# zkemail/zkemail.rs

Measured on AMD Instinct MI355X. Metric: emails verified/sec (witness gen), higher is better.
Workload: dtype u32; 1 GPU; BASELINE configs[1]: batch 1024 e-mails, 4 KB body, RSA-2048, DKIM-only verify_email; body_bytes=4096, rsa_bits=2048, algo=rsa-sha256, inputs=HBM-resident raw e-mails, batches_in_flight=22, collective=none

## Files before the change

### bindings/zkemail-amd-sys/src/lib.rs

```rust
#![allow(non_camel_case_types, non_upper_case_globals)]

use core::ffi::{c_char, c_int, c_void};

pub const ZKE_OK: u32 = 0;
pub const ZKE_PARSE_FAIL: u32 = 1;
pub const ZKE_KEY_DECODE_FAIL: u32 = 2;
pub const ZKE_DKIM_ERROR: u32 = 3;
pub const ZKE_DKIM_NOT_PASS: u32 = 4;
pub const ZKE_EXTERNAL_INPUT_NULL: u32 = 5;
pub const ZKE_CANON_FAIL: u32 = 6;
pub const ZKE_DFA_DECODE_FAIL: u32 = 7;
pub const ZKE_HEADER_REGEX_FAIL: u32 = 8;
pub const ZKE_BODY_REGEX_FAIL: u32 = 9;
pub const ZKE_UNSUPPORTED: u32 = 10;
pub const ZKE_BODY_DECODE_FAIL: u32 = 11;
pub const ZKE_D_NONE: u32 = 0;
pub const ZKE_D_NEUTRAL: u32 = 1;
pub const ZKE_D_SIG_SYNTAX: u32 = 2;
pub const ZKE_D_MISSING_TAG: u32 = 3;
pub const ZKE_D_INCOMPATIBLE_VERSION: u32 = 4;
pub const ZKE_D_DOMAIN_MISMATCH: u32 = 5;
pub const ZKE_D_FROM_NOT_SIGNED: u32 = 6;
pub const ZKE_D_BAD_QUERY_METHOD: u32 = 7;
pub const ZKE_D_BAD_CANON: u32 = 8;
// ... 437 lines not shown
    pub fn zke_select_keys(e: *mut zke_engine, emails: *const zke_email_ref, n: u32, cand_off: *const u32, keys: *const zke_key_ref, out: *mut zke_result, chosen: *mut u32) -> c_int;
    pub fn zke_select_keys_async(e: *mut zke_engine, emails: *const zke_email_ref, n: u32, cand_off: *const u32, keys: *const zke_key_ref, out: *mut zke_result, chosen: *mut u32, ticket: *mut u64) -> c_int;
    pub fn zke_decode_key_records(e: *mut zke_engine, recs: *const zke_keyrec_ref, m: u32, mode: u32, out: *mut zke_keyrec_out) -> c_int;
    pub fn zke_decode_key_records_async(e: *mut zke_engine, recs: *const zke_keyrec_ref, m: u32, mode: u32, out: *mut zke_keyrec_out, ticket: *mut u64) -> c_int;
    pub fn zke_select_keys_from_records(e: *mut zke_engine, emails: *const zke_email_ref, n: u32, cand_off: *const u32, recs: *const zke_keyrec_ref, mode: u32, out: *mut zke_result, chosen: *mut u32, keys_out: *mut zke_keyrec_out) -> c_int;
    pub fn zke_select_keys_from_records_async(e: *mut zke_engine, emails: *const zke_email_ref, n: u32, cand_off: *const u32, recs: *const zke_keyrec_ref, mode: u32, out: *mut zke_result, chosen: *mut u32, keys_out: *mut zke_keyrec_out, ticket: *mut u64) -> c_int;
    pub fn zke_extract_bodies(e: *mut zke_engine, emails: *const zke_email_ref, n: u32, flags: u32, out: *mut zke_body_out) -> c_int;
    pub fn zke_extract_bodies_async(e: *mut zke_engine, emails: *const zke_email_ref, n: u32, flags: u32, out: *mut zke_body_out, ticket: *mut u64) -> c_int;
    pub fn zke_verify_batch_device(e: *mut zke_engine, r#in: *const zke_batch, raw_total: u64, domain_total: u64, key_total: u64, out_dev: *mut zke_result, stream: *mut c_void) -> c_int;
    pub fn zke_engine_sync(e: *mut zke_engine) -> c_int;
    pub fn zke_engine_join(e: *mut zke_engine, stream: *mut c_void) -> c_int;
    pub fn zke_get_timings(e: *mut zke_engine, t: *mut zke_timings) -> c_int;
    pub fn zke_get_slot_timings(e: *mut zke_engine, slot: u32, t: *mut zke_timings) -> c_int;
    pub fn zke_engine_sha_ring(e: *mut zke_engine) -> c_int;
    pub fn zke_engine_sha_twin(e: *mut zke_engine) -> c_int;
    pub fn zke_set_timing(e: *mut zke_engine, enabled: c_int) -> c_int;
    pub fn zke_verify_email(e: *mut zke_engine, raw: *const u8, raw_len: usize, from_domain: *const c_char, domain_len: usize, key: *const u8, key_len: usize, key_type: u32, external_input_null: u32, out: *mut zke_result) -> c_int;
    pub fn zke_verify_email_with_regex(e: *mut zke_engine, raw: *const u8, raw_len: usize, from_domain: *const c_char, domain_len: usize, key: *const u8, key_len: usize, key_type: u32, external_input_null: u32, header_parts: *const zke_regex_part, n_header_parts: u32, body_parts: *const zke_regex_part, n_body_parts: u32, out: *mut zke_result) -> c_int;
    pub fn zke_wire_decode(format: u32, bytes: *const u8, len: usize, with_regex: u32, out: *mut *mut zke_wire_doc, consumed: *mut usize) -> c_int;
    pub fn zke_wire_free(d: *mut zke_wire_doc);
    pub fn zke_wire_view(d: *const zke_wire_doc, out: *mut zke_wire_email) -> c_int;
    pub fn zke_wire_external_input(d: *const zke_wire_doc, i: u32, name: *mut *const u8, name_len: *mut usize, value: *mut *const u8, value_len: *mut usize, is_null: *mut u32) -> c_int;
    pub fn zke_verify_wire(e: *mut zke_engine, format: u32, bytes: *const u8, len: usize, with_regex: u32, out: *mut zke_result) -> c_int;
    pub fn zke_shard_bounds(raw_off: *const u64, n: u32, world: u32, bounds: *mut u32) -> c_int;
    pub fn zke_sha256_batch(e: *mut zke_engine, msg_blob: *const u8, off: *const u64, n: u32, digests: *mut u8) -> c_int;
    pub fn zke_rsa_modexp_batch(e: *mut zke_engine, sig: *const u8, r#mod: *const u8, exp: *const u64, bytes: u32, n: u32, em: *mut u8, ok: *mut u8) -> c_int;
    pub fn zke_ed25519_verify_batch(e: *mut zke_engine, keys: *const u8, msgs: *const u8, msg_len: u32, sigs: *const u8, n: u32, out: *mut u32) -> c_int;
    pub fn zke_sha256_batch_device(e: *mut zke_engine, msg_blob_dev: *const u8, off_dev: *const u64, n: u32, digests_dev: *mut u8, stream: *mut c_void) -> c_int;
    pub fn zke_abi_encode(from_domain_hash: *const u8, public_key_hash: *const u8, external_inputs: *const *const u8, external_input_lens: *const usize, n_external_inputs: u32, with_matches: u32, matches: *const *const u8, match_lens: *const usize, n_matches: u32, out: *mut u8, out_cap: usize, out_len: *mut usize) -> c_int;
    pub fn zke_version() -> *const c_char;
// ... 5 lines not shown
```

### include/zkemail_amd.h

```cpp
#ifndef ZKEMAIL_AMD_H
#define ZKEMAIL_AMD_H

#include <stddef.h>
#include <stdint.h>

#ifdef __cplusplus
extern "C" {
#endif

enum {
  ZKE_OK                  = 0,
  ZKE_PARSE_FAIL          = 1,
  ZKE_KEY_DECODE_FAIL     = 2,
  ZKE_DKIM_ERROR          = 3,
  ZKE_DKIM_NOT_PASS       = 4,
  ZKE_EXTERNAL_INPUT_NULL = 5,
  ZKE_CANON_FAIL          = 6,
  ZKE_DFA_DECODE_FAIL     = 7,
  ZKE_HEADER_REGEX_FAIL   = 8,
  ZKE_BODY_REGEX_FAIL     = 9,
  ZKE_UNSUPPORTED         = 10,
  ZKE_BODY_DECODE_FAIL    = 11
};

// ... 353 lines not shown
  uint8_t*       bytes; size_t bytes_cap;
  size_t infos_need, bytes_need;
} zke_body_out;
int zke_extract_bodies(zke_engine* e, const zke_email_ref* emails, uint32_t n, uint32_t flags, zke_body_out* out);
int zke_extract_bodies_async(zke_engine* e, const zke_email_ref* emails, uint32_t n, uint32_t flags, zke_body_out* out, uint64_t* ticket);

int zke_verify_batch_device(zke_engine* e, const zke_batch* in, uint64_t raw_total,
                            uint64_t domain_total, uint64_t key_total,
                            zke_result* out_dev, void* stream);
int zke_engine_sync(zke_engine* e);
int zke_engine_join(zke_engine* e, void* stream);
int zke_get_timings(zke_engine* e, zke_timings* t);
int zke_get_slot_timings(zke_engine* e, uint32_t slot, zke_timings* t);
int zke_engine_sha_ring(zke_engine* e);
int zke_engine_sha_twin(zke_engine* e);
int zke_set_timing(zke_engine* e, int enabled);

int zke_verify_email(zke_engine* e, const uint8_t* raw, size_t raw_len,
                     const char* from_domain, size_t domain_len,
                     const uint8_t* key, size_t key_len, uint32_t key_type,
                     uint32_t external_input_null, zke_result* out);

typedef struct zke_regex_part {
  const uint8_t* fwd; size_t fwd_len;
  const uint8_t* bwd; size_t bwd_len;
  uint32_t n_captures;
  const uint8_t* const* captures;
  const size_t* capture_lens;
} zke_regex_part;

// ... 57 lines not shown
```

### zkemail.rs_amd/csrc/canon.hip.h

```cpp
#pragma once
#include "parse.hip.h"
#include <type_traits>

namespace zke {

__device__ __forceinline__ uint32_t ld_coherent_u8(const uint8_t* p) {
  return (uint32_t)__hip_atomic_load(p, __ATOMIC_RELAXED, __HIP_MEMORY_SCOPE_AGENT);
}

template <class LD>
__device__ __forceinline__ uint32_t trailing_crlf_pairs(LD load, uint32_t len, bool* ended = nullptr) {
  uint32_t matched = 0, pos = len;
  if (ended) *ended = false;
  while (pos > 0) {
    const uint32_t lo = pos > 64 ? pos - 64 : 0;
    const uint32_t l = lo + lane_id();
    bool bad = false;
    if (l < pos) {
      const uint32_t c = load(l);
      bad = c != (((len - 1 - l) & 1) ? (uint32_t)'\r' : (uint32_t)'\n');
    }
    const uint64_t m = __ballot(bad);
    if (m) { matched += (pos - 1) - (lo + 63u - (uint32_t)__builtin_clzll(m)); if (ended) *ended = true; break; }
    matched += pos - lo;
    pos = lo;
  }
  return matched / 2;
}

constexpr uint32_t CANON_LDS_TRASH = 3504, CANON_LDS_BYTES = 3504 + 64;
static_assert(CANON_LDS_BYTES <= PARSE_STAGE_BYTES, "the front end lends its staging buffer to the canonicaliser");
__device__ __forceinline__ void canon_body_wave(const BatchDev& B, uint32_t i, uint32_t mode, uint32_t flags, uint32_t boff,
                                                uint32_t blen, uint64_t len_tag, uint8_t* lds, bool ignore_l, bool bucket,
                                                uint32_t hdr_len) {
  const int lane = lane_id();
  EmailMeta* M = B.meta + i;
  zke_result* R = B.results + i;
  const uint64_t r0 = B.raw_off[i];
  const uint32_t raw_len = (uint32_t)(B.raw_off[i + 1] - r0);
  const uint8_t* body = B.raw + r0 + boff;
  uint8_t* regB = B.scratch + scratch_offset(r0 - B.raw_off[0], i) + (((size_t)raw_len + PRE_SLACK + 15) & ~(size_t)15);
  uint32_t full = 0, src_is_raw = 0;

  if (!(flags & ZKE_F_BODY_RELAXED)) {
    if (blen == 0) {
      if (lane < 2) regB[lane] = lane ? '\n' : '\r';
      full = 2;
    } else {
      const uint32_t m = trailing_crlf_pairs([&](uint32_t l) { return (uint32_t)body[l]; }, blen);
      full = m >= 2 ? blen - 2 * (m - 1) : blen;
      src_is_raw = 1;
    }
  } else {
    typedef uint32_t __attribute__((aligned(1))) u32_unaligned;
    typedef uint4 __attribute__((aligned(1))) uint4_store_unaligned;
    auto load4 = [&](uint32_t pos) -> uint32_t {
// ... 166 lines not shown
        }
        __builtin_amdgcn_fence(__ATOMIC_RELEASE, "wavefront");
        __builtin_amdgcn_wave_barrier();
        o += fill;
        fill = 0;
      }
    }
    if (!tail_done) {
      __builtin_amdgcn_fence(__ATOMIC_RELEASE, "agent");
      const uint32_t m = trailing_crlf_pairs([&](uint32_t l) { return ld_coherent_u8(regB + l); }, o);
      if (m >= 2) o -= 2 * (m - 1);
      else if (o > 0 && m == 0) { if (lane < 2) regB[o + lane] = lane ? '\n' : '\r'; o += 2; }
    }
    full = o;
  }
  uint32_t hashed = full;
  if ((flags & ZKE_F_HAS_LENGTH) && !ignore_l) {
    if (len_tag < hashed) hashed = (uint32_t)len_tag;
  }
  if (lane == 0) {
    M->canon_full_len = full; M->hashed_len = hashed; M->body_src_is_raw = src_is_raw;
    if (mode == 0) {
      R->canon_body_len = hashed;
      ShaJob j; j.src = (uint64_t)(src_is_raw ? body : regB); j.dst = (uint64_t)R->body_hash; j.len = hashed;
      j.pad = (flags & ZKE_F_SHA1) ? 1u : 0u;
      B.sha[i] = j;
    }
  }
  if (bucket && lane < 2) sha_bucket(B.order, (uint32_t)lane, B.n_pad, i, lane ? hdr_len : hashed);
}

struct FinArgs { BatchDev b; uint32_t round, max_rounds; uint32_t* pending; uint32_t debug_skip_rsa; };

constexpr uint32_t META_WORDS = sizeof(EmailMeta) / 4;
static_assert(sizeof(EmailMeta) % 16 == 0 && offsetof(EmailMeta, bh) % 4 == 0, "EmailMeta is read as 16-byte words (hipMalloc aligns the array)");
static_assert(offsetof(zke_result, header_hash) == offsetof(zke_result, body_hash) + 32, "the two hashes are read as one run of 16 words");
struct VerdictIn {
  uint32_t m[META_WORDS];
  uint32_t hash[16];
  uint32_t ext_null;
};
#define ZKE_MW(field) (offsetof(EmailMeta, field) / 4)
__device__ __forceinline__ void verdict_load(const EmailMeta* M, const zke_result* R, const uint8_t* ext, VerdictIn& V) {
  const uint4* mp = reinterpret_cast<const uint4*>(M);
// ... 90 lines not shown
```

### zkemail.rs_amd/csrc/engine.hip

```cpp
#include <hip/hip_runtime.h>
#include <hip/hip_ext.h>

#include <algorithm>
#include <atomic>
#include <cstddef>
#include <cstdio>
#include <cstdlib>
#include <cstring>
#include <ctime>
#include <mutex>
#include <shared_mutex>
#include <string>
#include <unordered_map>
#include <vector>

#include "zkemail_amd.h"
#include "sha256.hip.h"
#include "rsa.hip.h"
#include "parse.hip.h"
#include "regex.hip.h"
#include "capture.hip.h"
#include "qpmap.hip.h"
#include "sigscan.hip.h"
#include "keyrec.hip.h"
// ... 375 lines not shown
  delete e;
}

int zke_engine_sha_ring(zke_engine* e) {
  if (!e) return ZKE_E_ARG;
  std::shared_lock<std::shared_mutex> sh(e->big);
  return sha_takes_ring(e->stage) ? 1 : 0;
}

int zke_engine_sha_twin(zke_engine* e) {
  if (!e) return ZKE_E_ARG;
  std::shared_lock<std::shared_mutex> sh(e->big);
  return sha_takes_twin(e->stage) ? 1 : 0;
}

const char* zke_last_error(const zke_engine* e) { (void)e; return g_err.c_str(); }

int zke_engine_join(zke_engine* e, void* stream) {
  if (!e) return ZKE_E_ARG;
  std::shared_lock<std::shared_mutex> sh(e->big);
  HIPCHK(e, hipSetDevice(e->device));
  hipStream_t s = (hipStream_t)stream;
  for (Slot* w : e->slots) {
    std::lock_guard<std::mutex> g(w->mu);
    if (!w->last_stream) continue;
    if (w->last_stream == w->stream) {
      if (s == w->stream) continue;
      HIPCHK(e, hipEventRecord(w->done, w->stream));
    } else if (w->last_stream == s) {
      continue;
// ... 164 lines not shown
```

### zkemail.rs_amd/csrc/parse.hip.h

```cpp
#pragma once
#include <hip/hip_runtime.h>
#include <stdint.h>

#include "zkemail_amd.h"
#include "rsa.hip.h"
#include "sha256.hip.h"
#include "bytes.hip.h"
#include "taglist.hip.h"
#include "hdrsplit.hip.h"
#include "keydec.hip.h"

namespace zke {

struct EmailMeta {
  uint32_t state;
  uint32_t status, detail;
  uint32_t unsupported;
  uint32_t last_touched_sig;
  uint32_t cand_total;
  uint32_t cand_sig_index;
  uint32_t cand_hdr;
  uint32_t cand_err;
  uint32_t post_err;
  uint32_t pre_err;
// ... 89 lines not shown
  uint32_t debug_stop;
  uint32_t strict;
  uint64_t now;
  const KeyCacheEntry* cache;
  uint32_t route_mask;
  uint32_t* wave_count;
  uint32_t* wave_list;
};

#ifdef ZKE_DEV_KNOBS
#define ZKE_DEV_STOP(k) do { if (A.debug_stop == (k)) return; } while (0)
#else
#define ZKE_DEV_STOP(k) do { } while (0)
#endif

__device__ __forceinline__ void canon_body_wave(const BatchDev& B, uint32_t i, uint32_t mode, uint32_t flags, uint32_t boff,
                                                uint32_t blen, uint64_t len_tag, uint8_t* lds, bool ignore_l, bool bucket,
                                                uint32_t hdr_len = 0);
__device__ __forceinline__ void sha_bucket(uint32_t* order, uint32_t kind, uint32_t n_pad, uint32_t i, uint32_t len) {
  const uint32_t cls = sha_len_class((len + 9 + 63) >> 6);
  order[sha_order_key(kind, n_pad) + i] = (cls << 24) | (atomicAdd(order + sha_order_cnt(kind) + cls, 1u) & 0xFFFFFFu);
}


template <bool FAST = true, int MODE = 0>
__device__ __forceinline__ void parse_email(const ParseArgs& A, const uint32_t i, ParseLds& L) {
  const BatchDev& B = A.b;
  const int lane = lane_id();
  EmailMeta* M = B.meta + i;
  zke_result* R = B.results + i;
  RsaJob* J = B.rsa + i;
  const uint32_t round = A.round;
  if (round > 0 && MODE == 0) {
    if (lane < 4) { ShaJob z{0, 0, 0, 0}; B.sha[(size_t)lane * B.n_pad + i] = z; }
    if (lane == 0) J->flags = 0;
    if (M->state != ST_PENDING) return;
  }

  const uint64_t r0 = B.raw_off[i], r1 = B.raw_off[i + 1];
  if (round == 0 && MODE == 0) batch_prologue(B, i, lane == 0, i == 0, (uint32_t)lane, 64);
  Str raw = mkstr(B.raw + r0, (uint32_t)(r1 - r0));
// ... 157 lines not shown
      auto next_occurrence = [&](uint32_t from, uint32_t skip_at) -> uint32_t {
        for (uint32_t base = from; base + bl <= v.len; base += 64) {
          const uint32_t p = base + lane;
          bool cand = p + bl <= v.len && p != skip_at;
          for (uint32_t t = 0; t < fl && cand; t++) cand = ldb(v, p + t) == ldb(v, b_rs + t);
          uint64_t m = __ballot(cand);
          while (m) {
            const uint32_t q = base + (uint32_t)__builtin_ctzll(m);
            m &= m - 1;
            if (same_bytes(v, q, b_rs, bl)) return q;
          }
        }
        return NONE;
      };
      if (!(A.strict & ZKE_STRICT_B_OWN_SPAN) && next_occurrence(0, b_rs) != NONE) {
        uint32_t pos = 0;
        while (pos < v.len) {
          const uint32_t q = next_occurrence(pos, NONE);
          const uint32_t end = (q == NONE) ? v.len : q;
          for (uint32_t base = pos; base < end; base += 64) { const uint32_t l = base + (uint32_t)lane; if (l < end) tmp[tn + (l - pos)] = (uint8_t)ldb(v, l); }
          tn += end - pos;
          if (q == NONE) break;
          pos = q + bl;
        }
        __builtin_amdgcn_fence(__ATOMIC_RELEASE, "agent");
        __builtin_amdgcn_fence(__ATOMIC_ACQUIRE, "agent");
        copied = true;
      }
    }
    Str sv = v;
    if (copied) sv = mkstr(tmp, tn);
    else if (bl) { sv.len = v.len - bl; sv.cut = b_rs; sv.skip = bl; }
    ZKE_DEV_STOP(6);
    Out out{regA, 0, capA, false};
    const bool hrel = (flags & ZKE_F_HDR_RELAXED) != 0;
    const uint32_t hks_lane = hn.ks, hnl_lane = hn.nl;
    {
      const uint8_t* h = L.tagbuf + tagf(L, TG_H, 2);
      const uint32_t hl = tagf(L, TG_H, 3);
      const bool one_win = hl <= 64;
      const uint64_t colons = one_win ? __ballot((uint32_t)lane < hl && h[(uint32_t)lane < hl ? lane : 0] == ':') : 0ull;
      auto colon_after = [&](uint32_t from) -> uint32_t {
        if (one_win) { const uint64_t m = colons & bits_from(from); return m ? (uint32_t)__builtin_ctzll(m) : hl; }
        for (uint32_t base = from & ~63u; base < hl; base += 64) {
          const uint32_t l = base + (uint32_t)lane;
          const uint64_t m = __ballot(l < hl && l >= from && h[l] == ':');
          if (m) return base + (uint32_t)__builtin_ctzll(m);
        }
// ... 70 lines not shown
  if (!have_cand) {
    if (lane == 0) R->sig_index = last_touched;
    if (unsupported) finish(ZKE_UNSUPPORTED, unsupported);
    else finish(ZKE_DKIM_NOT_PASS, err_all ? err_all : (round == 0 ? ZKE_D_NEUTRAL : M->cand_err));
    return;
  }
  ZKE_DEV_STOP(7);
  if (lane == 0) {
    M->state = ST_CAND;
    const uint32_t jf = (cand_flags & ZKE_F_ED25519) ? 0u : (RSA_F_ACTIVE | ((cand_flags & ZKE_F_SHA1) ? (uint32_t)RSA_F_SHA1 : 0u) |
                                                                  (A.route_mask ? M->rsa_route & RSA_F_GROUPS : 0u));
    J->flags = jf;
    M->em_ok = 0;
    if ((jf & RSA_F_ACTIVE) && !(jf & RSA_F_GROUPS) && A.wave_list) A.wave_list[atomicAdd(A.wave_count, 1u)] = i;
  }
  canon_body_wave(B, i, 0, cand_flags, body_off, raw.len - body_off, cand_len_tag, L.stage, false, bucket, cand_hdr_len);
}

#ifndef ZKE_PARSE_PRIO
#define ZKE_PARSE_PRIO 3
#endif
#ifndef ZKE_PARSE_WAVES
#define ZKE_PARSE_WAVES 5
#endif
#ifndef ZKE_PARSE_WG_WAVES
#define ZKE_PARSE_WG_WAVES 1
#endif
constexpr size_t PARSE_DYN_LDS = ZKE_PARSE_WG_WAVES > 1 ? ZKE_PARSE_WG_WAVES * sizeof(ParseLds) : 0;
#ifdef ZKE_PARSE_NUM_VGPR
#define ZKE_PARSE_VGPR_ATTR __attribute__((amdgpu_num_vgpr(ZKE_PARSE_NUM_VGPR)))
#else
#define ZKE_PARSE_VGPR_ATTR
#endif
__global__ __launch_bounds__(64 * ZKE_PARSE_WG_WAVES, ZKE_PARSE_WAVES) ZKE_PARSE_VGPR_ATTR void parse_kernel(ParseArgs A) {
#if ZKE_PARSE_WG_WAVES > 1
  extern __shared__ __attribute__((aligned(16))) uint8_t parse_lds_raw[];
  ParseLds* L = reinterpret_cast<ParseLds*>(parse_lds_raw);
#else
  __shared__ ParseLds L[1];
#endif
  const uint32_t wave = ZKE_PARSE_WG_WAVES > 1 ? __builtin_amdgcn_readfirstlane(threadIdx.x >> 6) : 0;
  const uint32_t email = blockIdx.x * ZKE_PARSE_WG_WAVES + wave;
  if (email >= A.b.n) return;
  if (ZKE_PARSE_PRIO) __builtin_amdgcn_s_setprio(ZKE_PARSE_PRIO);
  parse_email(A, email, L[wave]);
}

__global__ void sha_jobs_from_csr_kernel(const uint8_t* blob, const uint64_t* off, uint32_t n, uint8_t* digests, ShaJob* jobs) {
  uint32_t i = blockIdx.x * blockDim.x + threadIdx.x;
  if (i >= n) return;
  ShaJob j;
  j.src = (uint64_t)(blob + off[i]);
  j.dst = (uint64_t)(digests + (size_t)i * 32);
  j.len = (uint32_t)(off[i + 1] - off[i]);
  j.pad = 0;
  jobs[i] = j;
}

}
```

### zkemail.rs_amd/csrc/pipeline.hip.h

```cpp
#pragma once

namespace {

struct StageTimer {
  Slot* w; hipStream_t s; bool on;
  StageTimer(zke_engine* e_, Slot* w_, hipStream_t s_) : w(w_), s(s_), on(e_->timing.load()) {}
  void mark(int k) { if (on && hipEventRecord(w->ev[k], s) == hipSuccess) w->marks |= 1u << k; }
};

int ensure_zeroed(DevBuf& b, size_t need, hipStream_t s) {
  const void* old = b.p;
  if (int r = b.ensure(need)) return r;
  if (b.p != old && hipMemsetAsync(b.p, 0, b.cap, s) != hipSuccess) return ZKE_E_DEVICE;
  return 0;
}

int ensure_workspace(zke_engine* e, Slot& w, uint32_t n, uint64_t raw_total, bool with_regex, uint32_t P, bool want_em, hipStream_t s) {
  const uint32_t n_pad = (n + 63) & ~63u;
  int r = 0;
  const size_t scratch_bytes = 2 * (size_t)raw_total + (size_t)(n + 1) * SCR_PER_EMAIL + 256;
  if ((r = w.meta.ensure((size_t)n * sizeof(EmailMeta))) || (r = w.rsa_jobs.ensure((size_t)n * sizeof(RsaJob))) ||
      (r = w.sha_jobs.ensure((size_t)4 * n_pad * sizeof(ShaJob))) || (r = w.rsa_ok.ensure((size_t)n * 4)) ||
      (r = ensure_zeroed(w.sha_order, (size_t)2 * (SHA_ORDER_KIND_WORDS + n_pad) * 4, s)) ||
      (r = w.scratch_off.ensure((size_t)(n + 1) * 16)) || (r = w.scratch.ensure(scratch_bytes)))
// ... 178 lines not shown
  B.n_pad = n_pad;
  B.scratch = w.scratch.as<uint8_t>();
  B.scratch_off = scratch_off;
  B.clean_off = clean_off;
  B.pending = w.pending.as<uint32_t>();
  B.meta_verify = nullptr;
  B.order = n < (1u << 24) ? w.sha_order.as<uint32_t>() : nullptr;

  const uint32_t rounds = e->opt.max_sig_rounds;
  const StagePlan plan = plan_stage(e->stage, n, 4 * n_pad, key_total > (uint64_t)n * 272, B.order != nullptr, __atomic_load_n(w.wave_feedback, __ATOMIC_RELAXED));
  {
    const uint32_t round = 0;
    uint32_t* wave_count = w.pending.as<uint32_t>() + 2;
    uint32_t* wave_list = w.rsa_ok.as<uint32_t>();
    ParseArgs pa{B, round, 0, e->debug_parse_stop, e->strict, now, e->key_cache.as<KeyCacheEntry>(), plan.route_mask, wave_count, wave_list};
    hipLaunchKernelGGL(parse_kernel, dim3((n + ZKE_PARSE_WG_WAVES - 1) / ZKE_PARSE_WG_WAVES), dim3(64 * ZKE_PARSE_WG_WAVES), PARSE_DYN_LDS, s, pa);
    tm.mark(MK_FRONT);
    if (!(e->debug_skip_launch & 1) &&
        (r = launch_hash_modexp(e, plan, B.sha, 4 * n_pad, B.rsa, n, B.meta, want_em ? w.em_dbg.as<uint8_t>() : nullptr, wave_count, wave_list, B.order, s)))
      return r;
    tm.mark(MK_HASH);
    EdVerdictArgs va{FinArgs{B, round, rounds, w.pending.as<uint32_t>(), e->debug_skip_rsa}, e->debug_skip_ed, wave_count,
                     e->key_cache.as<KeyCacheEntry>(), want_em ? w.em_dbg.as<uint8_t>() : nullptr, e->strict, now, w.wave_feedback};
    if (!(e->debug_skip_launch & 2)) hipLaunchKernelGGL(ed_verdict_kernel, dim3((n + VERDICT_EMAILS_PER_WAVE - 1) / VERDICT_EMAILS_PER_WAVE), dim3(64), 0, s, va);
    tm.mark(MK_VERDICT);
  }
  HIPCHK(e, hipGetLastError());

  if (in->with_regex) {
    PartInfo parts_small[16];
    std::vector<PartInfo> parts_big;
// ... 258 lines not shown
```

### zkemail.rs_amd/csrc/stage_plan.hip.h

```cpp
#pragma once
#include <stdint.h>
#include <stdlib.h>

#ifdef __HIP__
#define ZKE_PLAN_FN __host__ __device__ inline
#else
#define ZKE_PLAN_FN inline
#endif

namespace zke {

constexpr uint32_t ROUTE_QUAD = 1u;
constexpr uint32_t ROUTE_OCT = 2u;
constexpr uint32_t ROUTE_OCT9 = 4u;

enum class ShaRoutine : uint32_t {
  TWIN,
  RING,
  PAIR,
  BATCH,
};
constexpr uint32_t SHA_TWIN_WIDTH = 32;
ZKE_PLAN_FN uint32_t sha_routine_width(ShaRoutine r) {
  return r == ShaRoutine::BATCH ? 256u : r == ShaRoutine::TWIN ? SHA_TWIN_WIDTH : 64u;
// ... 12 lines not shown
  uint32_t kind = 0;
  for (; kind + 1 < SHA_KINDS; kind++) {
    const uint32_t g = sha_kind_groups(n_pad, twin_kinds, kind);
    if (b < g) break;
    b -= g;
  }
  return kind;
}

struct StageEnv {
  uint32_t slots = 0;
  uint32_t hw_queues = 4;
  int rsa_oct9 = -1;
  int sha_ring = -1;
  int sha_twin = -1;
  uint32_t twin_kinds = 3;
  uint32_t rsa_quad_min = 256;
  uint32_t rsa_oct_min = 128;
  uint32_t sha_mapping = 0;
  uint32_t rsa_lane_groups = 0;
  bool key_cache = false;
};

inline void stage_env_from_environment(StageEnv& v) {
  auto forced = [](const char* name, int& f) { if (const char* s = getenv(name)) f = atoi(s) != 0 ? 1 : 0; };
  const char* q = getenv("GPU_MAX_HW_QUEUES");
  const int hwq = q ? atoi(q) : 0;
  v.hw_queues = hwq > 0 ? (uint32_t)hwq : 4u;
  forced("ZKE_RSA_OCT9", v.rsa_oct9);
  forced("ZKE_SHA_RING", v.sha_ring);
  forced("ZKE_SHA_TWIN", v.sha_twin);
  if (const char* tk = getenv("ZKE_SHA_TWIN_KINDS")) v.twin_kinds = (uint32_t)atoi(tk) & 3u;
#ifdef ZKE_DEV_KNOBS
  if (const char* rm = getenv("ZKE_RSA_QUAD_MIN")) v.rsa_quad_min = (uint32_t)atoi(rm);
  if (const char* ro = getenv("ZKE_RSA_OCT_MIN")) v.rsa_oct_min = (uint32_t)atoi(ro);
#endif
}

inline uint32_t plan_min(uint32_t a, uint32_t b) { return a < b ? a : b; }
inline uint32_t plan_max(uint32_t a, uint32_t b) { return a > b ? a : b; }

constexpr uint32_t CHAIN_BOUND_IN_FLIGHT = 4;
inline bool chain_bound(const StageEnv& v) { return plan_min(v.slots, v.hw_queues) <= CHAIN_BOUND_IN_FLIGHT; }

constexpr uint32_t SHA_PAIR_MAX_GROUPS = 512;
inline bool sha_takes_pairs(const StageEnv& v, uint32_t groups) { return v.sha_mapping ? v.sha_mapping == 2 : groups <= SHA_PAIR_MAX_GROUPS; }
inline bool sha_takes_ring(const StageEnv& v) { return v.sha_ring >= 0 ? v.sha_ring == 1 : chain_bound(v); }
inline bool sha_takes_twin(const StageEnv& v) { return sha_takes_ring(v) && v.sha_twin != 0; }

inline uint32_t rsa_route_mask(const StageEnv& v, uint32_t n, bool any_big) {
  if (!v.key_cache || v.rsa_lane_groups == 1) return 0;
  const bool always = v.rsa_lane_groups == 2;
  const bool oct9 = v.rsa_oct9 >= 0 ? v.rsa_oct9 == 1 : !always && chain_bound(v);
  uint32_t m = 0;
  if (always || n >= v.rsa_quad_min) m |= oct9 ? ROUTE_OCT9 : ROUTE_QUAD;
  if (any_big && (always || n >= v.rsa_oct_min)) m |= ROUTE_OCT;
  return m;
}

struct ShaPlan { ShaRoutine routine; uint32_t grid; };
inline ShaPlan plan_sha(const StageEnv& v, uint32_t n) {
  const ShaRoutine r = !sha_takes_pairs(v, (n + 63) / 64) ? ShaRoutine::BATCH
                       : sha_takes_twin(v)               ? ShaRoutine::TWIN
                       : sha_takes_ring(v)               ? ShaRoutine::RING
                                                         : ShaRoutine::PAIR;
  const uint32_t w = sha_routine_width(r);
  return ShaPlan{r, (n + w - 1) / w};
}

#ifndef ZKE_WAVE_ROLE_MAX_GROUPS
#define ZKE_WAVE_ROLE_MAX_GROUPS 128
#endif
#ifndef ZKE_WAVE_ROLE_MIN_GROUPS
#define ZKE_WAVE_ROLE_MIN_GROUPS 8
#endif

struct StagePlan {
  uint32_t route_mask;
  ShaPlan front;
  ShaRoutine routine;
  uint32_t twin_kinds;
  uint32_t g_sha, g_wave, g_quad, g_oct, g_oct9;
  uint32_t grid() const { return g_sha + g_wave + g_quad + g_oct + g_oct9; }
};
inline StagePlan plan_stage(const StageEnv& v, uint32_t n, uint32_t n_sha, bool any_big, bool have_order, uint32_t last_wave_jobs) {
  StagePlan p{};
  p.route_mask = rsa_route_mask(v, n, any_big);
  const uint32_t want = last_wave_jobs == 0xFFFFFFFFu ? ZKE_WAVE_ROLE_MAX_GROUPS
                                                      : plan_max(ZKE_WAVE_ROLE_MIN_GROUPS, (plan_min(last_wave_jobs, n) + 1) / 2);
  p.g_wave = plan_min((n + 1) / 2, plan_min(want, ZKE_WAVE_ROLE_MAX_GROUPS));
  p.g_quad = (p.route_mask & ROUTE_QUAD) ? (n + 31) / 32 : 0;
  p.g_oct = (p.route_mask & ROUTE_OCT) ? (n + 15) / 16 : 0;
  p.g_oct9 = (p.route_mask & ROUTE_OCT9) ? (n + 15) / 16 : 0;
  p.routine = ShaRoutine::PAIR;
  const uint32_t groups = (n_sha + 63) / 64;
  if (!sha_takes_pairs(v, groups)) { p.front = plan_sha(v, n_sha); return p; }
  if (have_order && sha_takes_twin(v)) p.twin_kinds = v.twin_kinds;
  p.g_sha = p.twin_kinds ? sha_stage_groups(n_sha / 4, p.twin_kinds) : groups;
  if (p.g_sha) p.routine = p.twin_kinds ? ShaRoutine::TWIN : sha_takes_ring(v) ? ShaRoutine::RING : ShaRoutine::PAIR;
  return p;
}

// ... 2 lines not shown
```

### zkemail.rs_amd/engine.py

```python
from __future__ import annotations

import ctypes as C
import os
from typing import Callable, Dict, List, NamedTuple, Optional, Sequence, Tuple

import numpy as np

from . import _abi as A
from ._abi import (CompiledRegex, DebugBuffers, Email, EmailVerifierOutput, EmailWithRegex,
                   EmailWithRegexVerifierOutput, PackedBatch)

_PKG = os.path.dirname(os.path.abspath(__file__))
_LIB_PATH = os.environ.get("ZKE_LIB") or os.path.join(_PKG, "libzkemail_amd.so")
_lib = None


class EngineError(RuntimeError):
    """The C-ABI call itself failed (bad arguments, no device, library missing)."""


class VerifyPanic(AssertionError):

    def __init__(self, status: int, detail: int, index: int = 0):
        self.status, self.detail, self.index = status, detail, index
# ... 129 lines not shown
    lib.zke_select_keys_from_records.argtypes = [vp, erp, C.c_uint32, vp, krp, C.c_uint32, vp, vp, kop]
    lib.zke_select_keys_from_records.restype = C.c_int
    lib.zke_select_keys_from_records_async.argtypes = [vp, erp, C.c_uint32, vp, krp, C.c_uint32, vp, vp, kop, C.POINTER(C.c_uint64)]
    lib.zke_select_keys_from_records_async.restype = C.c_int
    bop = C.POINTER(A.zke_body_out)
    lib.zke_extract_bodies.argtypes = [vp, erp, C.c_uint32, C.c_uint32, bop]
    lib.zke_extract_bodies.restype = C.c_int
    lib.zke_extract_bodies_async.argtypes = [vp, erp, C.c_uint32, C.c_uint32, bop, C.POINTER(C.c_uint64)]
    lib.zke_extract_bodies_async.restype = C.c_int
    if hasattr(lib, "zke_engine_sha_ring"):
        lib.zke_engine_sha_ring.argtypes = [vp]
        lib.zke_engine_sha_ring.restype = C.c_int
    if hasattr(lib, "zke_engine_sha_twin"):
        lib.zke_engine_sha_twin.argtypes = [vp]
        lib.zke_engine_sha_twin.restype = C.c_int
    lib.zke_version.argtypes = []
    lib.zke_version.restype = C.c_char_p
    lib.zke_device_available.argtypes = []
    lib.zke_device_available.restype = C.c_int
    if path is None:
        _lib = lib
    return lib


EXPORTED_SYMBOLS = [
    "zke_engine_create", "zke_engine_destroy", "zke_last_error", "zke_dfa_register", "zke_verify_batch",
    "zke_verify_batch_device", "zke_engine_sync", "zke_get_timings", "zke_set_timing", "zke_verify_email",
    "zke_sha256_batch", "zke_sha256_batch_device", "zke_rsa_modexp_batch", "zke_version", "zke_device_available",
    "zke_ed25519_verify_batch", "zke_engine_reserve", "zke_get_slot_timings", "zke_verify_email_with_regex",
    "zke_abi_encode", "zke_engine_join", "zke_verify_batch_async", "zke_batch_wait", "zke_dfa_status", "zke_dfa_unregister",
    "zke_process_init", "zke_abi_version", "zke_engine_reserve_host", "zke_wire_decode", "zke_wire_free", "zke_wire_view",
    "zke_wire_external_input", "zke_verify_wire", "zke_shard_bounds", "zke_status_name", "zke_verify_emails", "zke_verify_emails_async",
    "zke_verify_emails_with_regex", "zke_verify_emails_with_regex_async",
    "zke_capture_validate", "zke_capture_register", "zke_capture_status", "zke_capture_unregister", "zke_extract_captures",
    "zke_extract_captures_async", "zke_capture_batch",
    "zke_scan_signatures", "zke_scan_signatures_async", "zke_select_keys", "zke_select_keys_async",
    "zke_decode_key_records", "zke_decode_key_records_async", "zke_select_keys_from_records", "zke_select_keys_from_records_async",
    "zke_engine_sha_ring", "zke_engine_sha_twin",
    "zke_qp_clean_batch", "zke_extract_captures_mapped", "zke_extract_captures_mapped_async",
    "zke_extract_bodies", "zke_extract_bodies_async",
]


class SigInfo(NamedTuple):
    header_index: int
    code: int
    algo: int
    selector: bytes
    value_span: Tuple[int, int]


class SigScan(NamedTuple):
    status: int
# ... 409 lines not shown
        self._check(self.lib.zke_engine_reserve_host(self.h, max_n, max_input_bytes), "zke_engine_reserve_host")

    def sync(self):
        self._check(self.lib.zke_engine_sync(self.h), "zke_engine_sync")

    def sha_ring(self) -> bool:
        r = self.lib.zke_engine_sha_ring(self.h)
        self._check(min(r, 0), "zke_engine_sha_ring")
        return r == 1

    def sha_twin(self) -> bool:
        r = self.lib.zke_engine_sha_twin(self.h)
        self._check(min(r, 0), "zke_engine_sha_twin")
        return r == 1

    def join(self, stream: int = 0):
        self._check(self.lib.zke_engine_join(self.h, stream), "zke_engine_join")

    def slot_timings(self, slot: int) -> dict:
        t = A.zke_timings()
        self._check(self.lib.zke_get_slot_timings(self.h, slot, C.byref(t)), "zke_get_slot_timings")
        return {k: getattr(t, k) for k, _ in A.zke_timings._fields_}

    def set_timing(self, on: bool):
        self._check(self.lib.zke_set_timing(self.h, 1 if on else 0), "zke_set_timing")

    def timings(self) -> dict:
        t = A.zke_timings()
        self._check(self.lib.zke_get_timings(self.h, C.byref(t)), "zke_get_timings")
        return {k: getattr(t, k) for k, _ in A.zke_timings._fields_}
# ... 274 lines not shown
```

Before: 16.27 million emails/s.

## Add a helper wave that canonicalises the body while the main wave parses headers

Measured after the change: 17.34 million emails/s, median of 6. +6.6%, better.

```diff
diff --git a/bindings/zkemail-amd-sys/src/lib.rs b/bindings/zkemail-amd-sys/src/lib.rs
--- a/bindings/zkemail-amd-sys/src/lib.rs
+++ b/bindings/zkemail-amd-sys/src/lib.rs
@@ -475,6 +475,7 @@
     pub fn zke_get_slot_timings(e: *mut zke_engine, slot: u32, t: *mut zke_timings) -> c_int;
     pub fn zke_engine_sha_ring(e: *mut zke_engine) -> c_int;
     pub fn zke_engine_sha_twin(e: *mut zke_engine) -> c_int;
+    pub fn zke_engine_front_helper(e: *mut zke_engine, n: u32) -> c_int;
     pub fn zke_set_timing(e: *mut zke_engine, enabled: c_int) -> c_int;
     pub fn zke_verify_email(e: *mut zke_engine, raw: *const u8, raw_len: usize, from_domain: *const c_char, domain_len: usize, key: *const u8, key_len: usize, key_type: u32, external_input_null: u32, out: *mut zke_result) -> c_int;
     pub fn zke_verify_email_with_regex(e: *mut zke_engine, raw: *const u8, raw_len: usize, from_domain: *const c_char, domain_len: usize, key: *const u8, key_len: usize, key_type: u32, external_input_null: u32, header_parts: *const zke_regex_part, n_header_parts: u32, body_parts: *const zke_regex_part, n_body_parts: u32, out: *mut zke_result) -> c_int;
diff --git a/include/zkemail_amd.h b/include/zkemail_amd.h
--- a/include/zkemail_amd.h
+++ b/include/zkemail_amd.h
@@ -391,6 +391,7 @@
 int zke_get_slot_timings(zke_engine* e, uint32_t slot, zke_timings* t);
 int zke_engine_sha_ring(zke_engine* e);
 int zke_engine_sha_twin(zke_engine* e);
+int zke_engine_front_helper(zke_engine* e, uint32_t n);
 int zke_set_timing(zke_engine* e, int enabled);
 
 int zke_verify_email(zke_engine* e, const uint8_t* raw, size_t raw_len,
diff --git a/zkemail.rs_amd/csrc/canon.hip.h b/zkemail.rs_amd/csrc/canon.hip.h
--- a/zkemail.rs_amd/csrc/canon.hip.h
+++ b/zkemail.rs_amd/csrc/canon.hip.h
@@ -28,18 +28,17 @@
   return matched / 2;
 }
 
-constexpr uint32_t CANON_LDS_TRASH = 3504, CANON_LDS_BYTES = 3504 + 64;
 static_assert(CANON_LDS_BYTES <= PARSE_STAGE_BYTES, "the front end lends its staging buffer to the canonicaliser");
-__device__ __forceinline__ void canon_body_wave(const BatchDev& B, uint32_t i, uint32_t mode, uint32_t flags, uint32_t boff,
-                                                uint32_t blen, uint64_t len_tag, uint8_t* lds, bool ignore_l, bool bucket,
-                                                uint32_t hdr_len) {
-  const int lane = lane_id();
-  EmailMeta* M = B.meta + i;
-  zke_result* R = B.results + i;
+__device__ __forceinline__ CanonWhere canon_where(const BatchDev& B, uint32_t i, uint32_t boff) {
   const uint64_t r0 = B.raw_off[i];
   const uint32_t raw_len = (uint32_t)(B.raw_off[i + 1] - r0);
-  const uint8_t* body = B.raw + r0 + boff;
-  uint8_t* regB = B.scratch + scratch_offset(r0 - B.raw_off[0], i) + (((size_t)raw_len + PRE_SLACK + 15) & ~(size_t)15);
+  return CanonWhere{B.raw + r0 + boff, B.scratch + scratch_offset(r0 - B.raw_off[0], i) + (((size_t)raw_len + PRE_SLACK + 15) & ~(size_t)15)};
+}
+__device__ __forceinline__ void canon_body_compute(const CanonWhere W, uint32_t flags, uint32_t blen, uint8_t* lds,
+                                                   uint32_t& full_out, uint32_t& src_is_raw_out) {
+  const int lane = lane_id();
+  const uint8_t* body = W.body;
+  uint8_t* regB = W.regB;
   uint32_t full = 0, src_is_raw = 0;
 
   if (!(flags & ZKE_F_BODY_RELAXED)) {
@@ -236,6 +235,16 @@
     }
     full = o;
   }
+  full_out = full; src_is_raw_out = src_is_raw;
+}
+
+__device__ __forceinline__ void canon_body_publish(const BatchDev& B, uint32_t i, const CanonWhere W, uint32_t mode, uint32_t flags, uint64_t len_tag,
+                                                   bool ignore_l, bool bucket, uint32_t hdr_len, uint32_t full, uint32_t src_is_raw) {
+  const int lane = lane_id();
+  EmailMeta* M = B.meta + i;
+  zke_result* R = B.results + i;
+  const uint8_t* body = W.body;
+  uint8_t* regB = W.regB;
   uint32_t hashed = full;
   if ((flags & ZKE_F_HAS_LENGTH) && !ignore_l) {
     if (len_tag < hashed) hashed = (uint32_t)len_tag;
@@ -250,6 +259,15 @@
     }
   }
   if (bucket && lane < 2) sha_bucket(B.order, (uint32_t)lane, B.n_pad, i, lane ? hdr_len : hashed);
+}
+
+__device__ __forceinline__ void canon_body_wave(const BatchDev& B, uint32_t i, uint32_t mode, uint32_t flags, uint32_t boff,
+                                                uint32_t blen, uint64_t len_tag, uint8_t* lds, bool ignore_l, bool bucket,
+                                                uint32_t hdr_len) {
+  uint32_t full, src_is_raw;
+  const CanonWhere W = canon_where(B, i, boff);
+  canon_body_compute(W, flags, blen, lds, full, src_is_raw);
+  canon_body_publish(B, i, W, mode, flags, len_tag, ignore_l, bucket, hdr_len, full, src_is_raw);
 }
 
 struct FinArgs { BatchDev b; uint32_t round, max_rounds; uint32_t* pending; uint32_t debug_skip_rsa; };
diff --git a/zkemail.rs_amd/csrc/engine.hip b/zkemail.rs_amd/csrc/engine.hip
--- a/zkemail.rs_amd/csrc/engine.hip
+++ b/zkemail.rs_amd/csrc/engine.hip
@@ -413,6 +413,12 @@
   return sha_takes_twin(e->stage) ? 1 : 0;
 }
 
+int zke_engine_front_helper(zke_engine* e, uint32_t n) {
+  if (!e) return ZKE_E_ARG;
+  std::shared_lock<std::shared_mutex> sh(e->big);
+  return ZKE_PARSE_HELPER && front_takes_helper(e->stage, n) ? 1 : 0;
+}
+
 const char* zke_last_error(const zke_engine* e) { (void)e; return g_err.c_str(); }
 
 int zke_engine_join(zke_engine* e, void* stream) {
diff --git a/zkemail.rs_amd/csrc/parse.hip.h b/zkemail.rs_amd/csrc/parse.hip.h
--- a/zkemail.rs_amd/csrc/parse.hip.h
+++ b/zkemail.rs_amd/csrc/parse.hip.h
@@ -127,17 +127,39 @@
 #define ZKE_DEV_STOP(k) do { } while (0)
 #endif
 
+constexpr uint32_t CANON_LDS_TRASH = 3504, CANON_LDS_BYTES = 3504 + 64;
 __device__ __forceinline__ void canon_body_wave(const BatchDev& B, uint32_t i, uint32_t mode, uint32_t flags, uint32_t boff,
                                                 uint32_t blen, uint64_t len_tag, uint8_t* lds, bool ignore_l, bool bucket,
                                                 uint32_t hdr_len = 0);
+struct CanonWhere { const uint8_t* body; uint8_t* regB; };
+__device__ __forceinline__ CanonWhere canon_where(const BatchDev& B, uint32_t i, uint32_t boff);
+__device__ __forceinline__ void canon_body_compute(const CanonWhere W, uint32_t flags, uint32_t blen, uint8_t* lds,
+                                                   uint32_t& full_out, uint32_t& src_is_raw_out);
+__device__ __forceinline__ void canon_body_publish(const BatchDev& B, uint32_t i, const CanonWhere W, uint32_t mode, uint32_t flags, uint64_t len_tag,
+                                                   bool ignore_l, bool bucket, uint32_t hdr_len, uint32_t full, uint32_t src_is_raw);
+
+struct HelperBox {
+  uint32_t go;
+  uint32_t flags, body_off, blen;
+  uint32_t len_tag_lo, len_tag_hi;
+  uint32_t full, src_is_raw;
+  uint32_t posted, joined;
+};
+
+__device__ __forceinline__ void wg_barrier() {
+  __builtin_amdgcn_fence(__ATOMIC_RELEASE, "workgroup");
+  __builtin_amdgcn_s_barrier();
+  __builtin_amdgcn_fence(__ATOMIC_ACQUIRE, "workgroup");
+}
 __device__ __forceinline__ void sha_bucket(uint32_t* order, uint32_t kind, uint32_t n_pad, uint32_t i, uint32_t len) {
   const uint32_t cls = sha_len_class((len + 9 + 63) >> 6);
   order[sha_order_key(kind, n_pad) + i] = (cls << 24) | (atomicAdd(order + sha_order_cnt(kind) + cls, 1u) & 0xFFFFFFu);
 }
 
 
-template <bool FAST = true, int MODE = 0>
-__device__ __forceinline__ void parse_email(const ParseArgs& A, const uint32_t i, ParseLds& L) {
+template <bool FAST = true, int MODE = 0, bool HELPER = false>
+__device__ __forceinline__ void parse_email(const ParseArgs& A, const uint32_t i, ParseLds& L, HelperBox* H = nullptr) {
+  static_assert(!HELPER || (FAST && MODE == 0), "the helper wave belongs to the round-0 verify front end");
   const BatchDev& B = A.b;
   const int lane = lane_id();
   EmailMeta* M = B.meta + i;
@@ -325,6 +347,12 @@
         return NONE;
       };
       if (!(A.strict & ZKE_STRICT_B_OWN_SPAN) && next_occurrence(0, b_rs) != NONE) {
+        if constexpr (HELPER) {
+          if (uni(H->posted)) {
+            if (!uni(H->joined)) wg_barrier();
+            if (lane == 0) { H->joined = 1; H->go = 0; }
+          }
+        }
         uint32_t pos = 0;
         while (pos < v.len) {
           const uint32_t q = next_occurrence(pos, NONE);
@@ -343,6 +371,17 @@
     if (copied) sv = mkstr(tmp, tn);
     else if (bl) { sv.len = v.len - bl; sv.cut = b_rs; sv.skip = bl; }
     ZKE_DEV_STOP(6);
+    if constexpr (HELPER) {
+      if (!uni(H->posted)) {
+        if (lane == 0) {
+          H->flags = flags; H->body_off = body_off; H->blen = raw.len - body_off;
+          H->len_tag_lo = (uint32_t)len_tag; H->len_tag_hi = (uint32_t)(len_tag >> 32);
+          H->go = copied ? 0u : 1u;
+          H->posted = 1;
+        }
+        wg_barrier();
+      }
+    }
     Out out{regA, 0, capA, false};
     const bool hrel = (flags & ZKE_F_HDR_RELAXED) != 0;
     const uint32_t hks_lane = hn.ks, hnl_lane = hn.nl;
@@ -443,7 +482,21 @@
     M->em_ok = 0;
     if ((jf & RSA_F_ACTIVE) && !(jf & RSA_F_GROUPS) && A.wave_list) A.wave_list[atomicAdd(A.wave_count, 1u)] = i;
   }
-  canon_body_wave(B, i, 0, cand_flags, body_off, raw.len - body_off, cand_len_tag, L.stage, false, bucket, cand_hdr_len);
+  if constexpr (HELPER) {
+    const bool posted = uni(H->posted) != 0;
+    if (posted && !uni(H->joined)) wg_barrier();
+    if (lane == 0 && posted) H->joined = 1;
+    uint32_t full, src_is_raw;
+    const CanonWhere W{raw.base + body_off, regA + (((size_t)raw.len + PRE_SLACK + 15) & ~(size_t)15)};
+    if (posted && uni(H->go) && uni(H->flags) == cand_flags && uni(H->len_tag_lo) == (uint32_t)cand_len_tag && uni(H->len_tag_hi) == (uint32_t)(cand_len_tag >> 32)) {
+      full = uni(H->full); src_is_raw = uni(H->src_is_raw);
+    } else {
+      canon_body_compute(W, cand_flags, raw.len - body_off, L.stage, full, src_is_raw);
+    }
+    canon_body_publish(B, i, W, 0, cand_flags, cand_len_tag, false, bucket, cand_hdr_len, full, src_is_raw);
+  } else {
+    canon_body_wave(B, i, 0, cand_flags, body_off, raw.len - body_off, cand_len_tag, L.stage, false, bucket, cand_hdr_len);
+  }
 }
 
 #ifndef ZKE_PARSE_PRIO
@@ -461,18 +514,52 @@
 #else
 #define ZKE_PARSE_VGPR_ATTR
 #endif
-__global__ __launch_bounds__(64 * ZKE_PARSE_WG_WAVES, ZKE_PARSE_WAVES) ZKE_PARSE_VGPR_ATTR void parse_kernel(ParseArgs A) {
+#ifndef ZKE_PARSE_HELPER
+#define ZKE_PARSE_HELPER 1
+#endif
+static_assert(sizeof(ParseLds) + CANON_LDS_BYTES + sizeof(HelperBox) == 10840, "LDS per workgroup of parse_kernel<true>: DESIGN §3, profiles/kernel_resource_usage.txt");
+template <bool HELPER>
+__global__ __launch_bounds__(HELPER ? 128 : 64 * ZKE_PARSE_WG_WAVES, ZKE_PARSE_WAVES) ZKE_PARSE_VGPR_ATTR void parse_kernel(ParseArgs A) {
+  if constexpr (HELPER) {
+    static_assert(!HELPER || ZKE_PARSE_WG_WAVES == 1, "the helper wave takes the place of a second e-mail in the workgroup");
+    __shared__ ParseLds L;
+    __shared__ __attribute__((aligned(16))) uint8_t canon_lds[CANON_LDS_BYTES];
+    __shared__ HelperBox box;
+    const uint32_t email = blockIdx.x;
+    if (email >= A.b.n) return;
+    if (ZKE_PARSE_PRIO) __builtin_amdgcn_s_setprio(ZKE_PARSE_PRIO);
+    const uint32_t wave = __builtin_amdgcn_readfirstlane(threadIdx.x >> 6);
+    if (wave == 0) {
+      if (lane_id() == 0) { box.posted = 0; box.joined = 0; }
+      parse_email<true, 0, true>(A, email, L, &box);
+      if (!uni(box.posted)) {
+        if (lane_id() == 0) box.go = 0;
+        wg_barrier();
+      }
+      if (!uni(box.joined)) wg_barrier();
+    } else {
+      wg_barrier();
+      if (uni(box.go)) {
+        uint32_t full, src_is_raw;
+        canon_body_compute(canon_where(A.b, email, uni(box.body_off)), uni(box.flags), uni(box.blen), canon_lds, full, src_is_raw);
+        if (lane_id() == 0) { box.full = full; box.src_is_raw = src_is_raw; }
+        asm volatile("s_waitcnt vmcnt(0)" ::: "memory");
+      }
+      wg_barrier();
+    }
+  } else {
 #if ZKE_PARSE_WG_WAVES > 1
-  extern __shared__ __attribute__((aligned(16))) uint8_t parse_lds_raw[];
-  ParseLds* L = reinterpret_cast<ParseLds*>(parse_lds_raw);
+    extern __shared__ __attribute__((aligned(16))) uint8_t parse_lds_raw[];
+    ParseLds* L = reinterpret_cast<ParseLds*>(parse_lds_raw);
 #else
-  __shared__ ParseLds L[1];
-#endif
-  const uint32_t wave = ZKE_PARSE_WG_WAVES > 1 ? __builtin_amdgcn_readfirstlane(threadIdx.x >> 6) : 0;
-  const uint32_t email = blockIdx.x * ZKE_PARSE_WG_WAVES + wave;
-  if (email >= A.b.n) return;
-  if (ZKE_PARSE_PRIO) __builtin_amdgcn_s_setprio(ZKE_PARSE_PRIO);
-  parse_email(A, email, L[wave]);
+    __shared__ ParseLds L[1];
+#endif
+    const uint32_t wave = ZKE_PARSE_WG_WAVES > 1 ? __builtin_amdgcn_readfirstlane(threadIdx.x >> 6) : 0;
+    const uint32_t email = blockIdx.x * ZKE_PARSE_WG_WAVES + wave;
+    if (email >= A.b.n) return;
+    if (ZKE_PARSE_PRIO) __builtin_amdgcn_s_setprio(ZKE_PARSE_PRIO);
+    parse_email(A, email, L[wave]);
+  }
 }
 
 __global__ void sha_jobs_from_csr_kernel(const uint8_t* blob, const uint64_t* off, uint32_t n, uint8_t* digests, ShaJob* jobs) {
diff --git a/zkemail.rs_amd/csrc/pipeline.hip.h b/zkemail.rs_amd/csrc/pipeline.hip.h
--- a/zkemail.rs_amd/csrc/pipeline.hip.h
+++ b/zkemail.rs_amd/csrc/pipeline.hip.h
@@ -216,7 +216,11 @@
     uint32_t* wave_count = w.pending.as<uint32_t>() + 2;
     uint32_t* wave_list = w.rsa_ok.as<uint32_t>();
     ParseArgs pa{B, round, 0, e->debug_parse_stop, e->strict, now, e->key_cache.as<KeyCacheEntry>(), plan.route_mask, wave_count, wave_list};
-    hipLaunchKernelGGL(parse_kernel, dim3((n + ZKE_PARSE_WG_WAVES - 1) / ZKE_PARSE_WG_WAVES), dim3(64 * ZKE_PARSE_WG_WAVES), PARSE_DYN_LDS, s, pa);
+#if ZKE_PARSE_HELPER
+    if (plan.front_helper) hipLaunchKernelGGL(parse_kernel<true>, dim3(n), dim3(128), 0, s, pa);
+    else
+#endif
+    hipLaunchKernelGGL(parse_kernel<false>, dim3((n + ZKE_PARSE_WG_WAVES - 1) / ZKE_PARSE_WG_WAVES), dim3(64 * ZKE_PARSE_WG_WAVES), PARSE_DYN_LDS, s, pa);
     tm.mark(MK_FRONT);
     if (!(e->debug_skip_launch & 1) &&
         (r = launch_hash_modexp(e, plan, B.sha, 4 * n_pad, B.rsa, n, B.meta, want_em ? w.em_dbg.as<uint8_t>() : nullptr, wave_count, wave_list, B.order, s)))
diff --git a/zkemail.rs_amd/csrc/stage_plan.hip.h b/zkemail.rs_amd/csrc/stage_plan.hip.h
--- a/zkemail.rs_amd/csrc/stage_plan.hip.h
+++ b/zkemail.rs_amd/csrc/stage_plan.hip.h
@@ -50,6 +50,7 @@
   int rsa_oct9 = -1;
   int sha_ring = -1;
   int sha_twin = -1;
+  int front_helper = -1;
   uint32_t twin_kinds = 3;
   uint32_t rsa_quad_min = 256;
   uint32_t rsa_oct_min = 128;
@@ -66,6 +67,7 @@
   forced("ZKE_RSA_OCT9", v.rsa_oct9);
   forced("ZKE_SHA_RING", v.sha_ring);
   forced("ZKE_SHA_TWIN", v.sha_twin);
+  forced("ZKE_FRONT_HELPER", v.front_helper);
   if (const char* tk = getenv("ZKE_SHA_TWIN_KINDS")) v.twin_kinds = (uint32_t)atoi(tk) & 3u;
 #ifdef ZKE_DEV_KNOBS
   if (const char* rm = getenv("ZKE_RSA_QUAD_MIN")) v.rsa_quad_min = (uint32_t)atoi(rm);
@@ -83,6 +85,11 @@
 inline bool sha_takes_pairs(const StageEnv& v, uint32_t groups) { return v.sha_mapping ? v.sha_mapping == 2 : groups <= SHA_PAIR_MAX_GROUPS; }
 inline bool sha_takes_ring(const StageEnv& v) { return v.sha_ring >= 0 ? v.sha_ring == 1 : chain_bound(v); }
 inline bool sha_takes_twin(const StageEnv& v) { return sha_takes_ring(v) && v.sha_twin != 0; }
+
+constexpr uint32_t FRONT_HELPER_MAX_BATCH = 1024;
+inline bool front_takes_helper(const StageEnv& v, uint32_t n) {
+  return v.front_helper >= 0 ? v.front_helper == 1 : chain_bound(v) && n <= FRONT_HELPER_MAX_BATCH;
+}
 
 inline uint32_t rsa_route_mask(const StageEnv& v, uint32_t n, bool any_big) {
   if (!v.key_cache || v.rsa_lane_groups == 1) return 0;
@@ -113,6 +120,7 @@
 
 struct StagePlan {
   uint32_t route_mask;
+  bool front_helper;
   ShaPlan front;
   ShaRoutine routine;
   uint32_t twin_kinds;
@@ -122,6 +130,7 @@
 inline StagePlan plan_stage(const StageEnv& v, uint32_t n, uint32_t n_sha, bool any_big, bool have_order, uint32_t last_wave_jobs) {
   StagePlan p{};
   p.route_mask = rsa_route_mask(v, n, any_big);
+  p.front_helper = front_takes_helper(v, n);
   const uint32_t want = last_wave_jobs == 0xFFFFFFFFu ? ZKE_WAVE_ROLE_MAX_GROUPS
                                                       : plan_max(ZKE_WAVE_ROLE_MIN_GROUPS, (plan_min(last_wave_jobs, n) + 1) / 2);
   p.g_wave = plan_min((n + 1) / 2, plan_min(want, ZKE_WAVE_ROLE_MAX_GROUPS));
diff --git a/zkemail.rs_amd/engine.py b/zkemail.rs_amd/engine.py
--- a/zkemail.rs_amd/engine.py
+++ b/zkemail.rs_amd/engine.py
@@ -167,6 +167,9 @@
     if hasattr(lib, "zke_engine_sha_twin"):
         lib.zke_engine_sha_twin.argtypes = [vp]
         lib.zke_engine_sha_twin.restype = C.c_int
+    if hasattr(lib, "zke_engine_front_helper"):
+        lib.zke_engine_front_helper.argtypes = [vp, C.c_uint32]
+        lib.zke_engine_front_helper.restype = C.c_int
     lib.zke_version.argtypes = []
     lib.zke_version.restype = C.c_char_p
     lib.zke_device_available.argtypes = []
@@ -189,7 +192,7 @@
     "zke_extract_captures_async", "zke_capture_batch",
     "zke_scan_signatures", "zke_scan_signatures_async", "zke_select_keys", "zke_select_keys_async",
     "zke_decode_key_records", "zke_decode_key_records_async", "zke_select_keys_from_records", "zke_select_keys_from_records_async",
-    "zke_engine_sha_ring", "zke_engine_sha_twin",
+    "zke_engine_sha_ring", "zke_engine_sha_twin", "zke_engine_front_helper",
     "zke_qp_clean_batch", "zke_extract_captures_mapped", "zke_extract_captures_mapped_async",
     "zke_extract_bodies", "zke_extract_bodies_async",
 ]
@@ -629,6 +632,11 @@
         self._check(min(r, 0), "zke_engine_sha_twin")
         return r == 1
 
+    def front_helper(self, n: int) -> bool:
+        r = self.lib.zke_engine_front_helper(self.h, n)
+        self._check(min(r, 0), "zke_engine_front_helper")
+        return r == 1
+
     def join(self, stream: int = 0):
         self._check(self.lib.zke_engine_join(self.h, stream), "zke_engine_join")
 
```
